# fpgasystems/GPU-FPGA-Recommendation-System

Hardware: AMD Instinct MI355X
Metric: inferences/sec at batch 256 (higher is better)
Workload: dtype f32; 1 GPU; Model-A (embedding_47_krnl: 47 tables, 1.415 GB) batch=256, fp32 FC 352-1024-512-256-1, all tables resident in one GPU's HBM; hash-filled tables, uniform per-table indices; index rows resident in HBM when the timed region starts (1024 rotating buffers), scores left in HBM (the bench contract's definition of `value`); value_pcie_inclusive = the reference's own loop (cuda_server.c:460-461,494-495): ; batch=256, driver_threads=2, workers_per_thread=2, batches_per_launch=64, parallelism=replicas x1

## Files before the change

### gpu-fpga-recommendation-system_amd/csrc/fr_api.cpp

```cpp
#include <chrono>
#include <cmath>
#include <cstdarg>
#include <cstdio>
#include <cstdlib>
#include <cstring>
#include <new>

#include "fr_internal.h"

static thread_local char g_err[512] = "";

void fr_set_error(const char *fmt, ...) {
    va_list ap;
    va_start(ap, fmt);
    vsnprintf(g_err, sizeof(g_err), fmt, ap);
    va_end(ap);
}

#ifdef FR_EXPERIMENTS
int fr_knob_env(const char *name, int dflt) {
    const char *e = getenv(name);
    return e ? atoi(e) : dflt;
}
#endif
// ... 1328 lines not shown
static int pipeline_flush(fr_worker *w) {
    while (w->n_active > 0) {
        int rc = pipeline_step(w);
        if (rc) return rc;
    }
    return FR_OK;
}

static int fused_group_initial() {
    const int g = FR_KNOB_ONCE("FUSED_GROUP", FR_FUSED_DEFAULT_BATCHES);
    return g < 1 ? 1 : (g > FR_FUSED_MAX_QUEUE ? FR_FUSED_MAX_QUEUE : g);
}
static int fused_group(const fr_ctx *c) { return c->stream_group.load(std::memory_order_relaxed); }

static bool fused_eligible(const fr_ctx *c) {
    const int enabled = FR_KNOB_ONCE("FUSED", 1);
    const int32_t *fc = c->model.fc;
    if (!enabled || c->n_shards != 1 || c->model.layout != FR_LAYOUT_SEMANTIC) return false;
    if (c->fc_precision == FR_FC_FP8) return frk_fused_f8_ok(fc[0], fc[1], fc[2], fc[3]);
    if (c->fc_precision == FR_FC_BF16) return frk_fused_h_ok(fc[0], fc[1], fc[2], fc[3]) || c->hk_ok == 1;
    return frk_fused_ok(fc[0], fc[1], fc[2], fc[3]);
}

extern "C" int fr_ctx_set_stream_group(fr_ctx *ctx, int batches_per_launch) {
    if (!ctx) FR_FAIL(FR_ERR_INVALID, "ctx is NULL");
    if (batches_per_launch < 1 || batches_per_launch > FR_FUSED_MAX_QUEUE)
        FR_FAIL(FR_ERR_INVALID, "batches_per_launch %d outside [1, %d]", batches_per_launch, FR_FUSED_MAX_QUEUE);
    ctx->stream_group.store(batches_per_launch, std::memory_order_relaxed);
    return FR_OK;
}

extern "C" int fr_ctx_set_small_block(fr_ctx *ctx, int max_batches) {
    if (!ctx) FR_FAIL(FR_ERR_INVALID, "ctx is NULL");
    if (max_batches < 0 || max_batches > 8) FR_FAIL(FR_ERR_INVALID, "max_batches %d outside [0, 8]", max_batches);
    ctx->small_block.store(max_batches, std::memory_order_relaxed);
    return FR_OK;
}

extern "C" int fr_ctx_stream_group(const fr_ctx *ctx) { return (ctx && !ctx->cpu && fused_eligible(ctx)) ? fused_group(ctx) : 1; }

static int fused_launch_slice(fr_worker *w, FrFusedArgs &a, int first, int n) {
    fr_ctx *c = w->ctx;
    const bool bf16 = c->fc_precision == FR_FC_BF16, fp8 = c->fc_precision == FR_FC_FP8;
    const int m2_forced = FR_KNOB_ONCE("FUSED_M2", -1);
    int tiles64 = 0;
    for (int i = 0; i < n; i++) tiles64 += (w->pending[first + i].batch + 63) / 64;
    const bool m2 = !bf16 && c->fc_precision == FR_FC_FP32 && frk_fused_m2_ok(c->model.fc[0], c->model.fc[1], c->model.fc[2], c->model.fc[3]) &&
                    (m2_forced == 1 || (m2_forced != 0 && fused_group(c) >= 64 && tiles64 > 128));
    const int per_wg = (bf16 || fp8) ? frk_fused_h_items_per_wg() : (m2 ? 64 : 32);
    int max_tiles = 0;
    for (int i = 0; i < n; i++) {
        a.b[i] = w->pending[first + i];
        const int tiles = (a.b[i].batch + per_wg - 1) / per_wg;
        if (tiles > max_tiles) max_tiles = tiles;
    }
    a.n_batches = n;
    a.tiles_per_batch = max_tiles;
    a.blist = nullptr;
    if (fp8) return frk_fused_f8_launch(a, w->stream);
    if (m2) return frk_fused_m2_launch(a, w->stream);
    if (bf16) return frk_fused_h_launch(a, w->stream);
    return frk_fused_launch(a, w->stream);
}

static int fused_flush(fr_worker *w) {
    if (w->n_pending == 0) return FR_OK;
    fr_ctx *c = w->ctx;
    FrFusedArgs a{};
    const bool bf16 = c->fc_precision == FR_FC_BF16, fp8 = c->fc_precision == FR_FC_FP8;
    a.words = c->d_words;
    a.n_words = c->n_words;
    a.idx_stride = (int)idx_cols(c);
    a.err_flag = w->d_err;
    if (fp8) {
        a.w1q = reinterpret_cast<const float4 *>(c->d_w_fp8[0]);
        a.w2q = reinterpret_cast<const float4 *>(c->d_w_fp8[1]);
        a.w3q = reinterpret_cast<const float4 *>(c->d_w_fp8[2]);
        a.wout = c->d_w[3];
        for (int l = 0; l < 3; l++) a.e_w[l] = c->f8_e_w[l];
        for (int l = 0; l < 4; l++) a.e_act[l] = c->f8_e_act[l];
    } else if (bf16) {
        a.w1q = reinterpret_cast<const float4 *>(c->d_w_bf16[0]);
        a.w2q = reinterpret_cast<const float4 *>(c->d_w_bf16[1]);
        a.w3q = reinterpret_cast<const float4 *>(c->d_w_bf16[2]);
        a.wout = reinterpret_cast<const float *>(c->d_w_bf16[3]);
    } else {
        a.w1q = reinterpret_cast<const float4 *>(c->d_wq[0]);
        a.w2q = reinterpret_cast<const float4 *>(c->d_wq[1]);
        a.w3q = reinterpret_cast<const float4 *>(c->d_wq[2]);
        a.wout = c->d_w[3];
    }
    a.K = c->model.fc[0];
    a.H1 = c->model.fc[1];
    a.H2 = c->model.fc[2];
    a.H3 = c->model.fc[3];
    a.stamps = g_stamp_buffer;
    const int n_all = w->n_pending;
    w->n_pending = 0;
    w->pending_items = 0;
    struct Keep {
        fr_worker *w;
        ~Keep() { keep_kernel(w); }
    } keep{w};
    if (bf16 || (fp8 && FR_KNOB_ONCE("FUSED_HK", -1) == 1 && c->d_w_fp8h[0] && c->d_w_fp8h[1] && c->d_w_fp8h[2])) {
        int tiles = 0, max_tiles = 0;
        for (int i = 0; i < n_all; i++) {
            const int t_ = (w->pending[i].batch + 63) / 64;
            tiles += t_;
            if (t_ > max_tiles) max_tiles = t_;
        }
        const int hk = FR_KNOB_ONCE("FUSED_HK", -1);
        const int hs_from = a.K <= 352 ? c->n_cu : c->n_cu + c->n_cu / 4;
        const bool only_hs = bf16 && !frk_fused_h_ok(a.K, a.H1, a.H2, a.H3);
        if (c->hk_ok == 1 && (only_hs || (hk != 0 && (hk == 1 || tiles >= hs_from)))) {
            if (!w->h_blist) {
                FR_HIP(hipHostMalloc((void **)&w->h_blist, sizeof(FrFusedBatch) * FR_FUSED_MAX_QUEUE * FR_BLIST_RING, hipHostMallocDefault));
                FR_HIP(hipMalloc((void **)&w->d_blist, sizeof(FrFusedBatch) * FR_FUSED_MAX_QUEUE * FR_BLIST_RING));
                for (int k = 0; k < FR_BLIST_RING; k++) FR_HIP(hipEventCreateWithFlags(&w->ev_blist[k], hipEventDisableTiming));
            }
            const int k = w->blist_cur;
            w->blist_cur = (k + 1) % FR_BLIST_RING;
            if (w->blist_busy[k]) FR_HIP(hipEventSynchronize(w->ev_blist[k]));
            FrFusedBatch *hb = w->h_blist + (size_t)k * FR_FUSED_MAX_QUEUE, *db = w->d_blist + (size_t)k * FR_FUSED_MAX_QUEUE;
            memcpy(hb, w->pending, sizeof(FrFusedBatch) * n_all);
            FR_HIP(hipMemcpyAsync(db, hb, sizeof(FrFusedBatch) * n_all, hipMemcpyHostToDevice, w->stream));
            FR_HIP(hipEventRecord(w->ev_blist[k], w->stream));
            w->blist_busy[k] = true;
            a.blist = db;
            a.n_batches = n_all;
            a.tiles_per_batch = max_tiles;
            if (bf16 && frk_fused_hk_takes_lp_rows(a.K) && lp_image_applies_hs(c)) {
                const int irc = lp_ensure_image(c, FR_FC_BF16);
                if (irc) return irc;
                a.words = c->d_words_lp;
                a.src_lp = 1;
            }
            if (bf16 && FR_KNOB_ONCE("FUSED_HS_ABLATE", 0)) a.e_act[3] = -776 - FR_KNOB_ONCE("FUSED_HS_ABLATE", 0);
            if (fp8) {
                a.w1q = reinterpret_cast<const float4 *>(c->d_w_fp8h[0]);
                a.w2q = reinterpret_cast<const float4 *>(c->d_w_fp8h[1]);
                a.w3q = reinterpret_cast<const float4 *>(c->d_w_fp8h[2]);
            }
            return frk_fused_hk_launch(a, c->n_cu, c->fc_precision, w->stream);
        }
    }
    for (int first = 0; first < n_all; first += FR_FUSED_MAX_BATCHES) {
        const int n = n_all - first < FR_FUSED_MAX_BATCHES ? n_all - first : FR_FUSED_MAX_BATCHES;
        int rc = fused_launch_slice(w, a, first, n);
        if (rc) return rc;
    }
    return FR_OK;
}

static int check_gather_args(fr_worker *w, const int32_t *d_idx, const float *d_dense) {
    fr_ctx *c = w->ctx;
    if (!d_idx) FR_FAIL(FR_ERR_INVALID, "d_idx is NULL");
    if (c->model.dense_len && !d_dense) FR_FAIL(FR_ERR_INVALID, "model has dense features but d_dense is NULL");
    return FR_OK;
}

static int launch_fc(fr_worker *w, int batch, const float *d_records, float *d_scores) {
    fr_ctx *c = w->ctx;
    if (c->n_shards > 1) FR_FAIL(FR_ERR_STATE, "fc on a sharded ctx needs the all-gathered records (use the sharded driver)");
    if (c->cpu) {
        frc_fc_chain(c->model.fc, c->d_w, d_records, batch, w->c_scratch, d_scores);
        return FR_OK;
    }
    if (w->n_active) FR_FAIL(FR_ERR_STATE, "pipeline busy: call fr_worker_sync first");
    if (w->launch_no == 0) w->launch_no = 1;
    const int ldm = round_up(batch, 32);
    const int par_prev = (int)((w->launch_no - 1) & 1);
    int rc;
    if (c->fc_precision == FR_FC_FP8) rc = frk_records_to_q16_fp8(d_records, act_set(w, par_prev).x, batch, c->model.fc[0], ldm, c->f8_e_act[0], w->stream);
    else if (c->fc_precision == FR_FC_BF16) rc = frk_records_to_q8_bf16(d_records, act_set(w, par_prev).x, batch, c->model.fc[0], ldm, w->stream);
    else rc = frk_transpose_records(d_records, act_set(w, par_prev).x, batch, c->model.fc[0], ldm, w->stream);
    if (rc) return rc;
    rc = pipeline_push(w, batch, 1, nullptr, nullptr, d_scores);
    if (rc) return rc;
    return pipeline_flush(w);
}

static int fc_from_slices_impl(fr_worker *w, int batch_total, int item0, int n_items, const float *d_gathered, float *d_scores, uint64_t *stage1_launch) {
    int rc = check_ready(w, n_items, false, true);
    if (rc) return rc;
    fr_ctx *c = w->ctx;
    if (!d_gathered || !d_scores) FR_FAIL(FR_ERR_INVALID, "NULL device pointer");
    if (batch_total < 1 || item0 < 0 || item0 + n_items > batch_total) FR_FAIL(FR_ERR_INVALID, "items [%d,+%d) outside batch %d", item0, n_items, batch_total);
    if (w->n_active || w->n_pending) FR_FAIL(FR_ERR_STATE, "pipeline busy: call fr_worker_sync first");
    if (c->cpu) {
        if (c->n_shards < 2) FR_FAIL(FR_ERR_STATE, "fc_from_slices needs a sharded context");
        frc_slices_to_records(d_gathered, c->n_shards, batch_total, c->slice_padded, c->shard_offset.data(), c->shard_len.data(), item0, n_items, w->c_x, c->model.fc[0]);
        frc_fc_chain(c->model.fc, c->d_w, w->c_x, n_items, w->c_scratch, d_scores);
        return FR_OK;
    }
    FR_SET_DEVICE(c);
    if (w->launch_no == 0) w->launch_no = 1;
    const int ldm = round_up(n_items, 32);
    const int par_prev = (int)((w->launch_no - 1) & 1);
    const int prec = w->calibrating ? (int)FR_FC_FP32 : c->fc_precision;
    float *xq = prec == FR_FC_FP32 ? act_set(w, par_prev).x : act_set(w, par_prev ^ 1).x;
    rc = frk_transpose_slices(d_gathered, c->n_shards, batch_total, c->slice_padded, c->shard_offset.data(), c->shard_len.data(), item0, n_items, xq, ldm,
                              w->stream);
    if (rc) return rc;
    if (prec != FR_FC_FP32) {
        rc = frk_q4_to_lp(prec, xq, act_set(w, par_prev).x, c->model.fc[0], ldm, c->f8_e_act[0], w->stream);
        if (rc) return rc;
    }
    if (stage1_launch) *stage1_launch = w->launch_no;
    rc = pipeline_push(w, n_items, 1, nullptr, nullptr, d_scores);
    if (rc) return rc;
    return pipeline_flush(w);
}

extern "C" int fr_worker_fc_from_slices(fr_worker *w, int batch_total, int item0, int n_items, const float *d_gathered, float *d_scores) {
    if (!w) FR_FAIL(FR_ERR_INVALID, "worker is NULL");
    int rc = fc_from_slices_impl(w, batch_total, item0, n_items, d_gathered, d_scores, nullptr);
    if (rc) return rc;
    w->in_flight = true;
    return FR_OK;
}

static int launch_pipeline(fr_worker *w, int batch, const int32_t *d_idx, const float *d_dense, float *d_scores) {
    fr_ctx *c = w->ctx;
    if (c->n_shards > 1) FR_FAIL(FR_ERR_STATE, "submit on a sharded ctx: use the sharded driver (gather_only + all-gather + fc_only)");
    if (c->cpu) {
        int rc = launch_gather(w, batch, d_idx, d_dense, w->d_records);
        if (rc) return rc;
        return launch_fc(w, batch, w->d_records, d_scores);
    }
    if (c->model.layout != FR_LAYOUT_SEMANTIC) {
        int rc = launch_gather(w, batch, d_idx, d_dense, w->d_records);
        if (rc) return rc;
        return launch_fc(w, batch, w->d_records, d_scores);
    }
    int rc = check_gather_args(w, d_idx, d_dense);
    if (rc) return rc;
    rc = pipeline_push(w, batch, 0, d_idx, d_dense, d_scores);
    if (rc) return rc;
    return pipeline_flush(w);
}

extern "C" int fr_worker_gather_only(fr_worker *w, int batch, const int32_t *d_idx, const float *d_dense, float *d_records) {
    int rc = check_ready(w, batch, true, false);
    if (rc) return rc;
    if (!d_records) FR_FAIL(FR_ERR_INVALID, "d_records is NULL");
    FR_SET_DEVICE(w->ctx);
    rc = launch_gather(w, batch, d_idx, d_dense, d_records);
    keep_kernel(w);
    if (rc) return rc;
    w->in_flight = true;
    return FR_OK;
}

extern "C" int fr_worker_gather_slices(fr_worker *w, int batch, const int32_t *d_idx, const float *d_dense, void *d_slice, int transport) {
    int rc = check_ready(w, batch, true, false);
    if (rc) return rc;
    if (!d_slice) FR_FAIL(FR_ERR_INVALID, "d_slice is NULL");
    if (transport != FR_FC_FP32 && transport != FR_FC_BF16 && transport != FR_FC_FP8) FR_FAIL(FR_ERR_INVALID, "bad transport %d", transport);
    if (transport != FR_FC_FP32 && w->ctx->model.layout != FR_LAYOUT_SEMANTIC) FR_FAIL(FR_ERR_STATE, "low-precision transport: SEMANTIC layout only");
    FR_SET_DEVICE(w->ctx);
    rc = launch_gather(w, batch, d_idx, d_dense, d_slice, transport);
    keep_kernel(w);
    if (rc) return rc;
    w->in_flight = true;
    return FR_OK;
}

extern "C" int fr_worker_fc_from_slices_lp(fr_worker *w, int batch_total, int item0, int n_items, const void *d_gathered, int transport, float *d_scores) {
    if (!w) FR_FAIL(FR_ERR_INVALID, "worker is NULL");
    if (transport == FR_FC_FP32) return fr_worker_fc_from_slices(w, batch_total, item0, n_items, reinterpret_cast<const float *>(d_gathered), d_scores);
    int rc = check_ready(w, n_items, false, true);
    if (rc) return rc;
    fr_ctx *c = w->ctx;
    if (transport != c->fc_precision) FR_FAIL(FR_ERR_STATE, "slice transport %d does not match the context's FC precision %d", transport, c->fc_precision);
    if (!d_gathered || !d_scores) FR_FAIL(FR_ERR_INVALID, "NULL device pointer");
    if (batch_total < 1 || item0 < 0 || item0 + n_items > batch_total) FR_FAIL(FR_ERR_INVALID, "items [%d,+%d) outside batch %d", item0, n_items, batch_total);
    if (w->n_active || w->n_pending) FR_FAIL(FR_ERR_STATE, "pipeline busy: call fr_worker_sync first");
    FR_SET_DEVICE(c);
    if (w->launch_no == 0) w->launch_no = 1;
    const int ldm = round_up(n_items, 32);
    const int par_prev = (int)((w->launch_no - 1) & 1);
    rc = frk_transpose_slices_lp(transport, d_gathered, c->n_shards, batch_total, c->slice_padded, c->shard_offset.data(), c->shard_len.data(), item0, n_items,
                                 act_set(w, par_prev).x, c->model.fc[0], ldm, w->stream);
    if (rc) return rc;
    rc = pipeline_push(w, n_items, 1, nullptr, nullptr, d_scores);
    if (rc) return rc;
    rc = pipeline_flush(w);
    if (rc) return rc;
    w->in_flight = true;
    return FR_OK;
}

extern "C" int fr_worker_fc_only(fr_worker *w, int batch, const float *d_records, float *d_scores) {
    int rc = check_ready(w, batch, false, true);
    if (rc) return rc;
    if (!d_records || !d_scores) FR_FAIL(FR_ERR_INVALID, "NULL device pointer");
    FR_SET_DEVICE(w->ctx);
    rc = launch_fc(w, batch, d_records, d_scores);
    if (rc) return rc;
    w->in_flight = true;
    return FR_OK;
}

extern "C" int fr_worker_fc_layer_only(fr_worker *w, int batch, int layer) {
    int rc = check_ready(w, batch, false, true);
    if (rc) return rc;
// ... 559 lines not shown
```

### gpu-fpga-recommendation-system_amd/csrc/fr_driver.cpp

```cpp
#include <atomic>
#include <chrono>
#include <cstring>
#include <mutex>
#include <thread>
#include <vector>

#include "fr_internal.h"

#define FR_DRAIN_DEVICE(ctx_)                          \
    do {                                               \
        if (!(ctx_)->cpu) {                            \
            FR_HIP(hipSetDevice((ctx_)->device));      \
            FR_HIP(hipDeviceSynchronize());            \
        }                                              \
    } while (0)

constexpr int FR_SCORE_RING = 512;

struct fr_driver {
    fr_ctx *ctx = nullptr;
    int n_threads = 0, depth = 0, max_batch = 0;
    std::vector<fr_worker *> workers;
    std::vector<std::vector<float>> host_rings;
    std::vector<float *> score_rings;
};

extern "C" void fr_driver_destroy(fr_driver *d) {
    if (!d) return;
    for (fr_worker *w : d->workers) fr_worker_destroy(w);
    if (d->ctx && !d->ctx->cpu) (void)hipSetDevice(d->ctx->device);
    for (float *p : d->score_rings) {
        if (p && d->ctx->cpu) free(p);
        else if (p) (void)hipFree(p);
    }
    fr_ctx *held = d->ctx;
    delete d;
    fr_ctx_unref(held);
}

extern "C" int fr_driver_create(fr_ctx *ctx, int n_threads, int depth, int max_batch, fr_driver **out) {
    if (!ctx || !out) FR_FAIL(FR_ERR_INVALID, "NULL argument");
    *out = nullptr;
    if (n_threads < 1 || n_threads > 256 || depth < 1 || depth > 64) FR_FAIL(FR_ERR_INVALID, "n_threads %d / depth %d out of range", n_threads, depth);
    fr_driver *d = new (std::nothrow) fr_driver();
    if (!d) FR_FAIL(FR_ERR_OOM, "out of host memory");
    d->ctx = ctx;
    fr_ctx_ref(ctx);
    d->n_threads = n_threads;
    d->depth = depth;
    d->max_batch = max_batch;
    for (int i = 0; i < n_threads * depth; i++) {
        fr_worker *w = nullptr;
        int rc = fr_worker_create(ctx, max_batch, &w);
        if (rc) {
            fr_driver_destroy(d);
            return rc;
        }
        d->workers.push_back(w);
        float *ring = nullptr;
        if (ctx->cpu) {
            ring = (float *)calloc((size_t)FR_SCORE_RING * max_batch, sizeof(float));
            if (!ring) {
                fr_driver_destroy(d);
                FR_FAIL(FR_ERR_OOM, "out of host memory (score ring)");
            }
            d->score_rings.push_back(ring);
            continue;
        }
        if (hipMalloc((void **)&ring, (size_t)FR_SCORE_RING * max_batch * sizeof(float)) != hipSuccess) {
            fr_driver_destroy(d);
            FR_FAIL(FR_ERR_OOM, "hipMalloc(score ring) failed");
        }
        (void)hipMemset(ring, 0, (size_t)FR_SCORE_RING * max_batch * sizeof(float));
        d->score_rings.push_back(ring);
    }
    {
        int expected = 0;
        const int w = n_threads * depth > 4 ? 4 : n_threads * depth;
        if (ctx->chain_width.compare_exchange_strong(expected, w, std::memory_order_relaxed)) ctx->chain_width_auto.store(false, std::memory_order_relaxed);
    }
    *out = d;
    return FR_OK;
}

extern "C" int fr_driver_run_resident(fr_driver *d, int batch, int64_t total_batches, const int32_t *const *d_idx_pool,
                                      const float *const *d_dense_pool, int n_pool, double *elapsed_s) {
    if (!d || !d_idx_pool || n_pool < 1 || !elapsed_s) FR_FAIL(FR_ERR_INVALID, "bad argument");
    if (batch < 1 || batch > d->max_batch || total_batches < 0) FR_FAIL(FR_ERR_INVALID, "batch %d / total %lld out of range", batch, (long long)total_batches);
    std::mutex mtx;
    int64_t global_batch_count = 0;
    std::vector<int> status(d->n_threads, FR_OK);
    std::vector<std::string> messages(d->n_threads);
    std::vector<std::thread> threads;
    FR_DRAIN_DEVICE(d->ctx);
    const auto t0 = std::chrono::steady_clock::now();
    for (int t = 0; t < d->n_threads; t++) {
        threads.emplace_back([&, t]() {
            fr_worker **wk = &d->workers[(size_t)t * d->depth];
            float **rings = &d->score_rings[(size_t)t * d->depth];
            int64_t local = 0;
            int rc = FR_OK;
#ifdef FR_EXPERIMENTS
            double t_push = 0.0, t_sync = 0.0, t_push_max = 0.0;
#endif
            while (rc == FR_OK) {
                int64_t id;
                {
                    std::lock_guard<std::mutex> g(mtx);
                    if (global_batch_count >= total_batches) break;
                    id = global_batch_count++;
                }
                const int slot = (int)(local % d->depth);
                float *scores = rings[slot] + (size_t)((local / d->depth) % FR_SCORE_RING) * d->max_batch;
                local++;
                const int p = (int)(id % n_pool);
#ifdef FR_EXPERIMENTS
                const auto tp0 = std::chrono::steady_clock::now();
#endif
                rc = fr_worker_push_device(wk[slot], batch, d_idx_pool[p], d_dense_pool ? d_dense_pool[p] : nullptr, scores);
#ifdef FR_EXPERIMENTS
                const auto tp1 = std::chrono::steady_clock::now();
                t_push += std::chrono::duration<double>(tp1 - tp0).count();
                const double dt = std::chrono::duration<double>(tp1 - tp0).count();
                if (dt > t_push_max) t_push_max = dt;
#endif
                const int64_t mine = (local - 1) / d->depth + 1;
                if (rc == FR_OK && (mine + (int64_t)slot * (FR_SCORE_RING / d->depth)) % FR_SCORE_RING == 0) rc = fr_worker_sync(wk[slot]);
#ifdef FR_EXPERIMENTS
                t_sync += std::chrono::duration<double>(std::chrono::steady_clock::now() - tp1).count();
#endif
            }
#ifdef FR_EXPERIMENTS
            if (FR_KNOB_ONCE("DRIVER_TIMING", 0))
                fprintf(stderr, "driver thread %d: %lld pushes, in push %.3f s (max %.1f us), in sync %.3f s\n", t, (long long)local, t_push, 1e6 * t_push_max, t_sync);
#endif
            for (int s = 0; s < d->depth; s++) {
                int r2 = fr_worker_sync(wk[s]);
                if (rc == FR_OK) rc = r2;
            }
            status[t] = rc;
            if (rc) messages[t] = fr_last_error();
        });
    }
    for (auto &th : threads) th.join();
    FR_DRAIN_DEVICE(d->ctx);
    *elapsed_s = std::chrono::duration<double>(std::chrono::steady_clock::now() - t0).count();
    for (int t = 0; t < d->n_threads; t++)
        if (status[t]) FR_FAIL(status[t], "driver thread %d: %s", t, messages[t].c_str());
    return FR_OK;
}

extern "C" int fr_driver_run_host(fr_driver *d, int batch, int64_t total_batches, const int32_t *const *h_idx_pool,
                                  const float *const *h_dense_pool, int n_pool, double *elapsed_s) {
    if (!d || !h_idx_pool || n_pool < 1 || !elapsed_s) FR_FAIL(FR_ERR_INVALID, "bad argument");
    if (batch < 1 || batch > d->max_batch || total_batches < 0) FR_FAIL(FR_ERR_INVALID, "batch %d / total %lld out of range", batch, (long long)total_batches);
    const fr_model_desc &m = d->ctx->model;
    const size_t idx_bytes = (size_t)batch * (size_t)fr_model_index_cols(&m) * sizeof(int32_t);
    const size_t dense_bytes = (size_t)batch * m.dense_len * sizeof(float);
    if (dense_bytes && !h_dense_pool) FR_FAIL(FR_ERR_INVALID, "model has dense features but h_dense_pool is NULL");
    std::mutex mtx;
    int64_t global_batch_count = 0;
    std::vector<int> status(d->n_threads, FR_OK);
    std::vector<std::string> messages(d->n_threads);
    std::vector<std::thread> threads;
    FR_DRAIN_DEVICE(d->ctx);
    const auto t0 = std::chrono::steady_clock::now();
    for (int t = 0; t < d->n_threads; t++) {
        threads.emplace_back([&, t]() {
            fr_worker **wk = &d->workers[(size_t)t * d->depth];
            std::vector<char> busy(d->depth, 0);
            int64_t local = 0;
            int rc = FR_OK;
            while (rc == FR_OK) {
                int64_t id;
                {
                    std::lock_guard<std::mutex> g(mtx);
                    if (global_batch_count >= total_batches) break;
                    id = global_batch_count++;
                }
                const int slot = (int)(local++ % d->depth);
                if (busy[slot]) {
                    rc = fr_worker_sync(wk[slot]);
                    busy[slot] = 0;
                    if (rc) break;
                }
                const int p = (int)(id % n_pool);
                memcpy(fr_worker_idx_ptr(wk[slot]), h_idx_pool[p], idx_bytes);
                if (dense_bytes) memcpy(fr_worker_dense_ptr(wk[slot]), h_dense_pool[p], dense_bytes);
                rc = fr_worker_submit(wk[slot], batch);
                if (rc == FR_OK) busy[slot] = 1;
            }
            for (int s = 0; s < d->depth; s++)
                if (busy[s]) {
                    int r2 = fr_worker_sync(wk[s]);
                    if (rc == FR_OK) rc = r2;
                }
            status[t] = rc;
            if (rc) messages[t] = fr_last_error();
        });
    }
    for (auto &th : threads) th.join();
    FR_DRAIN_DEVICE(d->ctx);
    *elapsed_s = std::chrono::duration<double>(std::chrono::steady_clock::now() - t0).count();
    for (int t = 0; t < d->n_threads; t++)
        if (status[t]) FR_FAIL(status[t], "driver thread %d: %s", t, messages[t].c_str());
    return FR_OK;
}

extern "C" int fr_driver_run_host_streaming(fr_driver *d, int batch, int64_t total_batches, const int32_t *const *h_idx_pool,
                                            const float *const *h_dense_pool, int n_pool, double *elapsed_s) {
    if (!d || !h_idx_pool || n_pool < 1 || !elapsed_s) FR_FAIL(FR_ERR_INVALID, "bad argument");
    if (batch < 1 || batch > d->max_batch || total_batches < 0) FR_FAIL(FR_ERR_INVALID, "batch %d / total %lld out of range", batch, (long long)total_batches);
    if (d->ctx->model.dense_len && !h_dense_pool) FR_FAIL(FR_ERR_INVALID, "model has dense features but h_dense_pool is NULL");
    FR_NOT_ON_CPU(d->ctx, "fr_driver_run_host_streaming");
    if (d->host_rings.empty()) {
        d->host_rings.resize(d->workers.size());
        for (auto &r : d->host_rings) r.assign((size_t)FR_SCORE_RING * d->max_batch, 0.0f);
    }
    std::mutex mtx;
    int64_t global_batch_count = 0;
    std::vector<int> status(d->n_threads, FR_OK);
    std::vector<std::string> messages(d->n_threads);
    std::vector<std::thread> threads;
    FR_DRAIN_DEVICE(d->ctx);
    const auto t0 = std::chrono::steady_clock::now();
    for (int t = 0; t < d->n_threads; t++) {
        threads.emplace_back([&, t]() {
            fr_worker **wk = &d->workers[(size_t)t * d->depth];
            int64_t local = 0;
            int rc = FR_OK;
            while (rc == FR_OK) {
                int64_t id;
                {
                    std::lock_guard<std::mutex> g(mtx);
                    if (global_batch_count >= total_batches) break;
                    id = global_batch_count++;
                }
                const int slot = (int)(local % d->depth);
                float *scores = d->host_rings[(size_t)t * d->depth + slot].data() + (size_t)((local / d->depth) % FR_SCORE_RING) * d->max_batch;
                local++;
                const int p = (int)(id % n_pool);
                rc = fr_worker_push_host(wk[slot], batch, h_idx_pool[p], h_dense_pool ? h_dense_pool[p] : nullptr, scores);
            }
            for (int s = 0; s < d->depth; s++) {
                int r2 = fr_worker_sync(wk[s]);
                if (rc == FR_OK) rc = r2;
            }
            status[t] = rc;
            if (rc) messages[t] = fr_last_error();
        });
    }
    for (auto &th : threads) th.join();
    FR_DRAIN_DEVICE(d->ctx);
    *elapsed_s = std::chrono::duration<double>(std::chrono::steady_clock::now() - t0).count();
    for (int t = 0; t < d->n_threads; t++)
        if (status[t]) FR_FAIL(status[t], "driver thread %d: %s", t, messages[t].c_str());
    return FR_OK;
}

extern "C" const float *fr_driver_host_score_ring(fr_driver *d, int thread, int slot, int *ring_len) {
    if (!d || thread < 0 || thread >= d->n_threads || slot < 0 || slot >= d->depth || d->host_rings.empty()) return nullptr;
    if (ring_len) *ring_len = FR_SCORE_RING;
    return d->host_rings[(size_t)thread * d->depth + slot].data();
}

extern "C" const float *fr_driver_score_ring(fr_driver *d, int thread, int slot, int *ring_len) {
    if (!d || thread < 0 || thread >= d->n_threads || slot < 0 || slot >= d->depth) return nullptr;
    if (ring_len) *ring_len = FR_SCORE_RING;
    return d->score_rings[(size_t)thread * d->depth + slot];
}

extern "C" fr_worker *fr_driver_worker(fr_driver *d, int thread, int slot) {
    if (!d || thread < 0 || thread >= d->n_threads || slot < 0 || slot >= d->depth) return nullptr;
    return d->workers[(size_t)thread * d->depth + slot];
}
```

### gpu-fpga-recommendation-system_amd/csrc/fr_internal.h

```cpp
#pragma once

#include <hip/hip_runtime.h>

#include <atomic>
#include <mutex>
#include <cstdint>
#include <string>
#include <vector>

#include "fleetrec.h"
#include "fleetrec_diag.h"
#include "fleetrec_serving.h"

void fr_set_error(const char *fmt, ...) __attribute__((format(printf, 1, 2)));

#define FR_FAIL(code, ...)         \
    do {                           \
        fr_set_error(__VA_ARGS__); \
        return (code);             \
    } while (0)

#define FR_HIP(call)                                                                                 \
    do {                                                                                             \
        hipError_t e_ = (call);                                                                      \
// ... 99 lines not shown
    int tiles_per_batch;
    const struct FrWordDesc *words;
    int src_lp;
    int n_words;
    int idx_stride;
    int *err_flag;
    const FrFusedBatch *blist;
    const float4 *w1q, *w2q, *w3q;
    const float *wout;
    int K, H1, H2, H3;
    int e_w[3], e_act[4];
    unsigned long long *stamps;
};

struct FrTableMem {
    uint64_t byte_offset = 0;
    uint64_t row_stride = 0;
    uint64_t il_rows = 0;
    uint64_t tail_offset = 0;
    bool resident = false;
};

struct fr_ctx {
    int device = -1;
    bool cpu = false;
    fr_model_desc model{};
    std::vector<fr_table_desc> tables;
    std::vector<fr_segment> segments;
    std::vector<FrTableMem> table_mem;
    std::vector<int> bank_of_table;
    std::vector<int64_t> bank_rows;
    int n_banks = 0;
    char *table_arena = nullptr;
    size_t table_arena_bytes = 0;
    bool tables_filled = false;
    int n_words = 0;
    FrWordDesc *d_words = nullptr;
    std::vector<FrWordDesc> h_words;
    FrGatherGroups gather_groups{};
    FrPassDesc *d_passes = nullptr;
    FrChunkDesc *d_chunks = nullptr;
    int n_chunks = 0;
    std::vector<int> h_word_table, h_word_col;
    char *lp_arena = nullptr;
    size_t lp_arena_bytes = 0;
    FrWordDesc *d_words_lp = nullptr;
    int lp_prec = 0, lp_e_x = 0;
    uint64_t lp_tables_gen = 0;
    uint64_t tables_gen = 1;
    std::mutex lp_mutex;
    std::atomic<int> lp_image_on{1};
    unsigned long long *d_merged = nullptr;
    std::atomic<int> gather_variant{0};
    float *d_w[4] = {nullptr, nullptr, nullptr, nullptr};
    float *d_wq[3] = {nullptr, nullptr, nullptr};
    uint16_t *d_w_bf16[4] = {nullptr, nullptr, nullptr, nullptr};
    void *d_w_fp8[3] = {nullptr, nullptr, nullptr};
    void *d_w_fp8h[3] = {nullptr, nullptr, nullptr};
    int f8_e_w[3] = {0, 0, 0};
    int f8_e_act[4] = {0, 0, 0, 0};
    float f8_w_rms_gain[3] = {1.0f, 1.0f, 1.0f};
    bool f8_calibrated = false;
    uint32_t *d_stats = nullptr;
    bool weights_set = false;
    int fc_precision = FR_FC_FP32;
    int shard_rank = 0, n_shards = 1;
    int slice_offset = 0, slice_len = 0, slice_padded = 0;
    std::vector<int> shard_offset, shard_len;
    hipStream_t setup_stream = nullptr;
    std::atomic<int> stream_group{FR_FUSED_DEFAULT_BATCHES};
    std::atomic<int> small_block{0};
    int n_cu = 0;
    int hk_ok = 0;
    std::atomic<int> life{1};
    std::atomic<int> n_workers{0};
    std::atomic<int> worker_seq{0};
    std::atomic<int> chain_width{0};
    std::atomic<bool> chain_width_auto{false};
};

struct fr_worker {
    fr_ctx *ctx = nullptr;
    int max_batch = 0;
    float *c_scratch = nullptr;
    float *c_x = nullptr;
    int c_err = 0;
    double c_t0 = 0.0;
    hipStream_t stream = nullptr;
    int32_t *h_idx = nullptr;
    float *h_dense = nullptr;
    float *h_score = nullptr;
    int32_t *d_idx = nullptr;
    float *d_dense = nullptr;
    float *d_records = nullptr;
    float *d_act[2] = {nullptr, nullptr};
    int ld_max = 0;
    struct Slot {
        bool active = false;
        uint64_t launch0 = 0;
        int first_stage = 0;
        int batch = 0, ldm = 0;
        const int32_t *d_idx = nullptr;
        const float *d_dense = nullptr;
        float *d_scores = nullptr;
    } ring[8];
    hipStream_t aux = nullptr;
    hipEvent_t ev_x_ready[2] = {nullptr, nullptr}, ev_x_free[2] = {nullptr, nullptr};
    bool x_ready_set[2] = {false, false}, x_free_set[2] = {false, false};
    uint64_t launch_no = 0;
    int n_active = 0;
    bool counted = false;
    bool diag_launch = false;
    bool calibrating = false;
    int last_x_parity = 0;
    FrFusedBatch pending[FR_FUSED_MAX_QUEUE];
    int n_pending = 0;
    FrFusedBatch *h_blist = nullptr, *d_blist = nullptr;
    hipEvent_t ev_blist[FR_BLIST_RING] = {nullptr, nullptr, nullptr, nullptr};
    bool blist_busy[FR_BLIST_RING] = {false, false, false, false};
    int blist_cur = 0;
    int64_t pending_items = 0;
    float *d_score = nullptr;
    struct HostRing {
        int g = 0;
        size_t idx_slot = 0, dense_slot = 0, score_slot = 0;
        int32_t *h_idx = nullptr, *d_idx = nullptr;
        float *h_dense = nullptr, *d_dense = nullptr, *h_sc = nullptr, *d_sc = nullptr;
        hipEvent_t ev[4] = {nullptr, nullptr, nullptr, nullptr};
        hipStream_t copy = nullptr;
        hipEvent_t ev_in[4] = {nullptr, nullptr, nullptr, nullptr};
        bool inflight[4] = {false, false, false, false};
        int count[4] = {0, 0, 0, 0};
        float *dst[4][FR_FUSED_MAX_BATCHES];
        int bsz[4][FR_FUSED_MAX_BATCHES];
        int cur = 0;
        int staged = 0;
        long long delivered = 0;
    } hr;
    void *d_slice = nullptr, *d_gathered = nullptr;
    float *d_score_part = nullptr, *d_score_all = nullptr;
    float *h_sh_status = nullptr;
    struct fr_comm *sh_comm = nullptr;
    int sh_ranks = 0;
    std::atomic<int> sh_inject_fc_fail{0};
    void *h_stage_send = nullptr, *h_stage_recv = nullptr;
    void *sh_host_stream = nullptr;
    int *h_err = nullptr;
    int *d_err = nullptr;
    bool in_flight = false;
    char last_kernel[96] = "";
    hipEvent_t ev_start = nullptr, ev_stop = nullptr;
};

void fr_ctx_ref(fr_ctx *c);
void fr_ctx_unref(fr_ctx *c);

int fr_comm_wait(fr_worker *w);
bool fr_comm_step_on_host_stream(const fr_worker *w);
void fr_comm_worker_release(fr_worker *w);
void fr_comm_forget(fr_worker *w);

int frc_set_threads(int n);
int frc_threads();
void *frc_arena_alloc(size_t bytes);
void frc_arena_free(void *p, size_t bytes);
int frc_fill_table(float *base, int64_t row0, int64_t rows, int dim, int64_t row_stride_bytes, int mode, uint32_t seed, uint32_t uid);
int frc_fill_weights(float *w, size_t count, int mode, uint32_t seed, uint32_t layer, float scale);
int frc_gather(const FrWordDesc *words, int n_words, const int32_t *idx, int idx_stride, const float *dense, float *out, int batch, int *err_flag);
void frc_fc_chain(const int32_t fc[5], const float *const w[4], const float *X, int batch, float *scratch, float *scores);
void frc_slices_to_records(const float *gathered, int n_shards, int batch_total, int slice_padded, const int *offs, const int *lens, int item0, int n_items, float *X, int K);
#define FR_NOT_ON_CPU(ctx_, what)                                                                                                  \
    do {                                                                                                                           \
        if ((ctx_)->cpu) FR_FAIL(FR_ERR_STATE, "%s is not available on the CPU back-end (device = -1): fp32 submit / sync / gather_only / fc_only only", what); \
    } while (0)

int fr_model_validate(const fr_model_desc *m);

static inline uint32_t fr_table_uid(const fr_table_desc &t) {
    return (uint32_t)t.source * 1024u + (uint32_t)t.mem_class * 256u + (uint32_t)t.table_id;
}
int frk_fill_table(float *base, int64_t row0, int64_t rows, int dim, int64_t row_stride_bytes, int mode, uint32_t seed, uint32_t uid, hipStream_t s);
int frk_fill_weights(float *w, size_t count, int mode, uint32_t seed, uint32_t layer, float scale, hipStream_t s);
int frk_convert_rows_lp(int precision, const void *src, size_t src_stride, void *dst, size_t dst_stride, int64_t rows, int floats, int e_x, hipStream_t s);
int frk_gather(const FrWordDesc *words, int n_words, const FrGatherGroups &groups, const int32_t *idx, int idx_stride, const float *dense, void *out, int batch, int *err_flag,
               int transport, int e_x, hipStream_t s, int out_words, bool one_chunk = false);
int frk_gather_tile(const FrPassDesc *passes, const FrChunkDesc *chunks, int n_chunks, const int32_t *idx, int idx_stride, const float *dense, void *out,
                    int out_stride_words, int batch, int *err_flag, bool dedup, unsigned long long *dup_counter, hipStream_t s);
int frk_transpose_slices_lp(int precision, const void *gathered, int n_shards, int batch_total, int slice_padded, const int *h_offsets, const int *h_lens,
                            int item0, int n_items, void *X, int K, int ldm, hipStream_t s);
int frk_pipeline_launch(const FrPipeArgs &a, int single_stage, int precision, hipStream_t s);
int frk_pack_weights_q8_bf16(const float *W, uint16_t *Wh, int K, int H, hipStream_t s);
bool frk_fc_lp_gemm_ok(int precision, int K, int N, int ldm);
int frk_fc_lp_gemm(int precision, const void *Wp, const void *Xp, void *Yp, int K, int N, int ldm, int e_w, int e_in, int e_out, int width, bool minor, hipStream_t s);
bool frk_fused_hk_takes_lp_rows(int K);
bool frk_fc_gemm_gather_ok(int precision, int K, int N, int ldm);
int frk_fc_gemm_gather(int precision, const void *Wp, const void *Xp, void *Yp, int K, int N, int ldm, int e_w, int e_in, int e_out, const FrWordDesc *words, int n_words,
                       int idx_stride, const int32_t *idx, const float *dense, int g_batch, int g_ldm, int g_K, void *g_out, int g_e_x, int *err_flag, hipStream_t s);
bool frk_fc_tail_ok(int precision, int K, int N, int ldm);
int frk_fc_tail(int precision, const void *W3, const void *R2, const void *wout, float *scores, int K, int N, int ldm, int batch, int e_w, int e_in, int e_r3, hipStream_t s);
int frk_records_to_q8_bf16(const float *X, void *Xh, int batch, int K, int ldm, hipStream_t s);
int frk_pack_weights_q16_fp8(const float *W, void *Wf, int K, int H, int e_w, hipStream_t s);
int frk_pack_weights_q16h_fp8(const float *W, void *Wg, int K, int H, int e_w, hipStream_t s);
int frk_records_to_q16_fp8(const float *X, void *Xf, int batch, int K, int ldm, int e_x, hipStream_t s);
int frk_stats(const float *p, size_t n, void *d_out, hipStream_t s);
int frk_q4_to_lp(int precision, const float *Xq, void *Xo, int K, int ldm, int e_x, hipStream_t s);
int frk_stage_blocks_f8_gather(int K, int ldm);
int frk_pack_weights_q4(const float *W, float *Wq, int K, int H, hipStream_t s);
int frk_stage_blocks(int stage, int n_words, int K, int N, int ldm, int nsplit);
int frk_gather_tr_blocks(int n_words, int ldm, int variant);
int frk_gather_tr_variant(int batch, int idx_stride);
bool frk_fused_ok(int K, int H1, int H2, int H3);
int frk_fused_launch(const FrFusedArgs &a, hipStream_t s);
bool frk_fused_m2_ok(int K, int H1, int H2, int H3);
int frk_fused_m2_launch(const FrFusedArgs &a, hipStream_t s);
bool frk_fused_h_ok(int K, int H1, int H2, int H3);
bool frk_fused_f8_ok(int K, int H1, int H2, int H3);
int frk_fused_f8_launch(const FrFusedArgs &a, hipStream_t s);
int frk_fused_h_items_per_wg();
int frk_fused_h_launch(const FrFusedArgs &a, hipStream_t s);
bool frk_fused_hk_ok(int K, int H1, int H2, int H3, const FrWordDesc *h_words, int n_words);
int frk_fused_hk_launch(const FrFusedArgs &a, int n_cu, int precision, hipStream_t s);
int frk_transpose_records(const float *X, float *Xt, int batch, int K, int ldm, hipStream_t s);
int frk_transpose_slices(const float *gathered, int n_shards, int batch_total, int slice_padded, const int *h_offsets, const int *h_lens,
                         int item0, int n_items, float *Xq, int ldm, hipStream_t s);
void fr_shard_bounds(const fr_model_desc &m, int n_shards, std::vector<int> &seg_begin);
int fr_bank_map(const fr_model_desc &m, std::vector<int> &bank_of_table, std::vector<int64_t> &bank_min_rows);
```

Measured before the change: 69.51 million inferences/s.

## Reuse persistent driver thread pool and merge worker tails into one flush

Replaces per-run std::thread creation with a persistent spin-then-sleep thread pool owned by the driver. The global batch counter becomes a lock-free atomic. At the end of a resident run, one thread gathers every worker's pending partial batches and relaunches them in full-size fused launches, instead of each worker flushing its own short tail. This targets thread startup latency, mutex contention and small tail launches inside the timed region, at the cost of spinning host threads and more complex end-of-run coordination.

```diff
diff --git a/gpu-fpga-recommendation-system_amd/csrc/fr_api.cpp b/gpu-fpga-recommendation-system_amd/csrc/fr_api.cpp
--- a/gpu-fpga-recommendation-system_amd/csrc/fr_api.cpp
+++ b/gpu-fpga-recommendation-system_amd/csrc/fr_api.cpp
@@ -1504,6 +1504,32 @@
     return FR_OK;
 }
 
+int fr_fused_flush_merged(fr_worker *const *ws, int n) {
+    int total = 0;
+    for (int i = 0; i < n; i++) total += ws[i]->n_pending;
+    if (total == 0) return FR_OK;
+    FR_SET_DEVICE(ws[0]->ctx);
+    std::vector<FrFusedBatch> all;
+    all.reserve((size_t)total);
+    for (int i = 0; i < n; i++) {
+        fr_worker *w = ws[i];
+        all.insert(all.end(), w->pending, w->pending + w->n_pending);
+        w->n_pending = 0;
+        w->pending_items = 0;
+    }
+    for (int first = 0, k = 0; first < total; first += FR_FUSED_MAX_BATCHES, k++) {
+        fr_worker *w = ws[k % n];
+        const int cnt = total - first < FR_FUSED_MAX_BATCHES ? total - first : FR_FUSED_MAX_BATCHES;
+        memcpy(w->pending, all.data() + first, sizeof(FrFusedBatch) * cnt);
+        w->n_pending = cnt;
+        for (int i = 0; i < cnt; i++) w->pending_items += w->pending[i].batch;
+        w->in_flight = true;
+        const int rc = fused_flush(w);
+        if (rc) return rc;
+    }
+    return FR_OK;
+}
+
 static int check_gather_args(fr_worker *w, const int32_t *d_idx, const float *d_dense) {
     fr_ctx *c = w->ctx;
     if (!d_idx) FR_FAIL(FR_ERR_INVALID, "d_idx is NULL");
diff --git a/gpu-fpga-recommendation-system_amd/csrc/fr_driver.cpp b/gpu-fpga-recommendation-system_amd/csrc/fr_driver.cpp
--- a/gpu-fpga-recommendation-system_amd/csrc/fr_driver.cpp
+++ b/gpu-fpga-recommendation-system_amd/csrc/fr_driver.cpp
@@ -1,6 +1,8 @@
 #include <atomic>
 #include <chrono>
+#include <condition_variable>
 #include <cstring>
+#include <functional>
 #include <mutex>
 #include <thread>
 #include <vector>
@@ -17,16 +19,84 @@
 
 constexpr int FR_SCORE_RING = 512;
 
+constexpr int FR_POOL_SPIN_US = 2000;
+
+template <typename Pred>
+static bool spin_until(Pred pred) {
+    const auto t_end = std::chrono::steady_clock::now() + std::chrono::microseconds(FR_POOL_SPIN_US);
+    for (;;) {
+        for (int i = 0; i < 64; i++) {
+            if (pred()) return true;
+            std::this_thread::yield();
+        }
+        if (std::chrono::steady_clock::now() >= t_end) return pred();
+    }
+}
+
+struct DriverPool {
+    std::mutex mtx;
+    std::condition_variable wake, done;
+    std::atomic<const std::function<void(int)> *> job{nullptr};
+    std::atomic<uint64_t> gen{0};
+    std::atomic<int> busy{0};
+    std::atomic<bool> stop{false};
+    std::vector<std::thread> threads;
+
+    void loop(int t) {
+        uint64_t seen = 0;
+        for (;;) {
+            auto ready = [&] { return stop.load(std::memory_order_acquire) || gen.load(std::memory_order_acquire) != seen; };
+            if (!spin_until(ready)) {
+                std::unique_lock<std::mutex> g(mtx);
+                wake.wait(g, ready);
+            }
+            if (stop.load(std::memory_order_acquire)) return;
+            seen = gen.load(std::memory_order_acquire);
+            (*job.load(std::memory_order_acquire))(t);
+            if (busy.fetch_sub(1, std::memory_order_acq_rel) == 1) {
+                std::lock_guard<std::mutex> g(mtx);
+                done.notify_one();
+            }
+        }
+    }
+    void run(const std::function<void(int)> &fn) {
+        job.store(&fn, std::memory_order_relaxed);
+        busy.store((int)threads.size(), std::memory_order_relaxed);
+        {
+            std::lock_guard<std::mutex> g(mtx);
+            gen.fetch_add(1, std::memory_order_release);
+        }
+        wake.notify_all();
+        auto finished = [&] { return busy.load(std::memory_order_acquire) == 0; };
+        if (!spin_until(finished)) {
+            std::unique_lock<std::mutex> g(mtx);
+            done.wait(g, finished);
+        }
+    }
+    void shutdown() {
+        {
+            std::lock_guard<std::mutex> g(mtx);
+            stop.store(true, std::memory_order_release);
+        }
+        wake.notify_all();
+        for (auto &th : threads) th.join();
+        threads.clear();
+    }
+};
+
 struct fr_driver {
     fr_ctx *ctx = nullptr;
     int n_threads = 0, depth = 0, max_batch = 0;
     std::vector<fr_worker *> workers;
     std::vector<std::vector<float>> host_rings;
     std::vector<float *> score_rings;
+    DriverPool pool;
+    std::mutex run_mtx;
 };
 
 extern "C" void fr_driver_destroy(fr_driver *d) {
     if (!d) return;
+    d->pool.shutdown();
     for (fr_worker *w : d->workers) fr_worker_destroy(w);
     if (d->ctx && !d->ctx->cpu) (void)hipSetDevice(d->ctx->device);
     for (float *p : d->score_rings) {
@@ -79,6 +149,12 @@
         const int w = n_threads * depth > 4 ? 4 : n_threads * depth;
         if (ctx->chain_width.compare_exchange_strong(expected, w, std::memory_order_relaxed)) ctx->chain_width_auto.store(false, std::memory_order_relaxed);
     }
+    try {
+        for (int t = 0; t < n_threads; t++) d->pool.threads.emplace_back([d, t]() { d->pool.loop(t); });
+    } catch (const std::exception &e) {
+        fr_driver_destroy(d);
+        FR_FAIL(FR_ERR_OOM, "cannot start the driver's host threads: %s", e.what());
+    }
     *out = d;
     return FR_OK;
 }
@@ -87,15 +163,17 @@
                                       const float *const *d_dense_pool, int n_pool, double *elapsed_s) {
     if (!d || !d_idx_pool || n_pool < 1 || !elapsed_s) FR_FAIL(FR_ERR_INVALID, "bad argument");
     if (batch < 1 || batch > d->max_batch || total_batches < 0) FR_FAIL(FR_ERR_INVALID, "batch %d / total %lld out of range", batch, (long long)total_batches);
-    std::mutex mtx;
-    int64_t global_batch_count = 0;
+    std::lock_guard<std::mutex> run_guard(d->run_mtx);
+    std::atomic<int64_t> global_batch_count{0};
+    std::atomic<int64_t> n_done{0};
+    std::atomic<int> n_out{0};
+    std::atomic<bool> tail_taken{false};
     std::vector<int> status(d->n_threads, FR_OK);
     std::vector<std::string> messages(d->n_threads);
-    std::vector<std::thread> threads;
     FR_DRAIN_DEVICE(d->ctx);
     const auto t0 = std::chrono::steady_clock::now();
-    for (int t = 0; t < d->n_threads; t++) {
-        threads.emplace_back([&, t]() {
+    {
+        const std::function<void(int)> job = [&](int t) {
             fr_worker **wk = &d->workers[(size_t)t * d->depth];
             float **rings = &d->score_rings[(size_t)t * d->depth];
             int64_t local = 0;
@@ -103,13 +181,12 @@
 #ifdef FR_EXPERIMENTS
             double t_push = 0.0, t_sync = 0.0, t_push_max = 0.0;
 #endif
+#ifdef FR_EXPERIMENTS
+            if (FR_KNOB_ONCE("DRIVER_TIMING", 0)) fprintf(stderr, "driver thread %d: job at +%.1f us\n", t, 1e6 * std::chrono::duration<double>(std::chrono::steady_clock::now() - t0).count());
+#endif
             while (rc == FR_OK) {
-                int64_t id;
-                {
-                    std::lock_guard<std::mutex> g(mtx);
-                    if (global_batch_count >= total_batches) break;
-                    id = global_batch_count++;
-                }
+                const int64_t id = global_batch_count.fetch_add(1, std::memory_order_relaxed);
+                if (id >= total_batches) break;
                 const int slot = (int)(local % d->depth);
                 float *scores = rings[slot] + (size_t)((local / d->depth) % FR_SCORE_RING) * d->max_batch;
                 local++;
@@ -129,20 +206,35 @@
 #ifdef FR_EXPERIMENTS
                 t_sync += std::chrono::duration<double>(std::chrono::steady_clock::now() - tp1).count();
 #endif
+                if (n_done.fetch_add(1, std::memory_order_acq_rel) + 1 == total_batches) break;
             }
 #ifdef FR_EXPERIMENTS
             if (FR_KNOB_ONCE("DRIVER_TIMING", 0))
-                fprintf(stderr, "driver thread %d: %lld pushes, in push %.3f s (max %.1f us), in sync %.3f s\n", t, (long long)local, t_push, 1e6 * t_push_max, t_sync);
-#endif
-            for (int s = 0; s < d->depth; s++) {
-                int r2 = fr_worker_sync(wk[s]);
-                if (rc == FR_OK) rc = r2;
-            }
+                fprintf(stderr, "driver thread %d: %lld pushes, in push %.3f s (max %.1f us), in sync %.3f s, out of ids at +%.1f us (cpu %d)\n", t, (long long)local, t_push,
+                        1e6 * t_push_max, t_sync, 1e6 * std::chrono::duration<double>(std::chrono::steady_clock::now() - t0).count(), sched_getcpu());
+#endif
+            if (rc) messages[t] = fr_last_error();
+            const bool last_batch = n_done.load(std::memory_order_acquire) == total_batches;
+            const bool last_out = n_out.fetch_add(1, std::memory_order_acq_rel) + 1 == d->n_threads;
+            if (!((last_batch || last_out) && !tail_taken.exchange(true, std::memory_order_acq_rel))) {
+                status[t] = rc;
+                return;
+            }
+            auto note = [&](int r) {
+                if (r && rc == FR_OK) {
+                    rc = r;
+                    messages[t] = fr_last_error();
+                }
+            };
+            note(fr_fused_flush_merged(d->workers.data(), (int)d->workers.size()));
+#ifdef FR_EXPERIMENTS
+            if (FR_KNOB_ONCE("DRIVER_TIMING", 0)) fprintf(stderr, "driver thread %d: tail launched at +%.1f us\n", t, 1e6 * std::chrono::duration<double>(std::chrono::steady_clock::now() - t0).count());
+#endif
+            for (fr_worker *w : d->workers) note(fr_worker_sync(w));
             status[t] = rc;
-            if (rc) messages[t] = fr_last_error();
-        });
-    }
-    for (auto &th : threads) th.join();
+        };
+        d->pool.run(job);
+    }
     FR_DRAIN_DEVICE(d->ctx);
     *elapsed_s = std::chrono::duration<double>(std::chrono::steady_clock::now() - t0).count();
     for (int t = 0; t < d->n_threads; t++)
@@ -158,15 +250,15 @@
     const size_t idx_bytes = (size_t)batch * (size_t)fr_model_index_cols(&m) * sizeof(int32_t);
     const size_t dense_bytes = (size_t)batch * m.dense_len * sizeof(float);
     if (dense_bytes && !h_dense_pool) FR_FAIL(FR_ERR_INVALID, "model has dense features but h_dense_pool is NULL");
+    std::lock_guard<std::mutex> run_guard(d->run_mtx);
     std::mutex mtx;
     int64_t global_batch_count = 0;
     std::vector<int> status(d->n_threads, FR_OK);
     std::vector<std::string> messages(d->n_threads);
-    std::vector<std::thread> threads;
     FR_DRAIN_DEVICE(d->ctx);
     const auto t0 = std::chrono::steady_clock::now();
-    for (int t = 0; t < d->n_threads; t++) {
-        threads.emplace_back([&, t]() {
+    {
+        const std::function<void(int)> job = [&](int t) {
             fr_worker **wk = &d->workers[(size_t)t * d->depth];
             std::vector<char> busy(d->depth, 0);
             int64_t local = 0;
@@ -197,9 +289,9 @@
                 }
             status[t] = rc;
             if (rc) messages[t] = fr_last_error();
-        });
-    }
-    for (auto &th : threads) th.join();
+        };
+        d->pool.run(job);
+    }
     FR_DRAIN_DEVICE(d->ctx);
     *elapsed_s = std::chrono::duration<double>(std::chrono::steady_clock::now() - t0).count();
     for (int t = 0; t < d->n_threads; t++)
@@ -213,6 +305,7 @@
     if (batch < 1 || batch > d->max_batch || total_batches < 0) FR_FAIL(FR_ERR_INVALID, "batch %d / total %lld out of range", batch, (long long)total_batches);
     if (d->ctx->model.dense_len && !h_dense_pool) FR_FAIL(FR_ERR_INVALID, "model has dense features but h_dense_pool is NULL");
     FR_NOT_ON_CPU(d->ctx, "fr_driver_run_host_streaming");
+    std::lock_guard<std::mutex> run_guard(d->run_mtx);
     if (d->host_rings.empty()) {
         d->host_rings.resize(d->workers.size());
         for (auto &r : d->host_rings) r.assign((size_t)FR_SCORE_RING * d->max_batch, 0.0f);
@@ -221,11 +314,10 @@
     int64_t global_batch_count = 0;
     std::vector<int> status(d->n_threads, FR_OK);
     std::vector<std::string> messages(d->n_threads);
-    std::vector<std::thread> threads;
     FR_DRAIN_DEVICE(d->ctx);
     const auto t0 = std::chrono::steady_clock::now();
-    for (int t = 0; t < d->n_threads; t++) {
-        threads.emplace_back([&, t]() {
+    {
+        const std::function<void(int)> job = [&](int t) {
             fr_worker **wk = &d->workers[(size_t)t * d->depth];
             int64_t local = 0;
             int rc = FR_OK;
@@ -248,9 +340,9 @@
             }
             status[t] = rc;
             if (rc) messages[t] = fr_last_error();
-        });
-    }
-    for (auto &th : threads) th.join();
+        };
+        d->pool.run(job);
+    }
     FR_DRAIN_DEVICE(d->ctx);
     *elapsed_s = std::chrono::duration<double>(std::chrono::steady_clock::now() - t0).count();
     for (int t = 0; t < d->n_threads; t++)
diff --git a/gpu-fpga-recommendation-system_amd/csrc/fr_internal.h b/gpu-fpga-recommendation-system_amd/csrc/fr_internal.h
--- a/gpu-fpga-recommendation-system_amd/csrc/fr_internal.h
+++ b/gpu-fpga-recommendation-system_amd/csrc/fr_internal.h
@@ -275,6 +275,8 @@
     hipEvent_t ev_start = nullptr, ev_stop = nullptr;
 };
 
+int fr_fused_flush_merged(fr_worker *const *ws, int n);
+
 void fr_ctx_ref(fr_ctx *c);
 void fr_ctx_unref(fr_ctx *c);
 
```

Measured after the change: 69.47 million inferences/s (median of 3 runs). About the same (-0.0%).
